# posgraph/coupe.optical_flow_based_deep_video_stabilization

Measured on AMD Instinct MI355X. Metric: stabilised frame-pairs/sec @512x512, higher is better.
Workload: dtype f32; 1 GPU; batch=8 512x512x27 frame stacks per GPU: FlowNetS-pyramid forward (5 flows) + flow resize/scale + tf_warp at 512x512; batch_per_gpu=8, height=512, width=512, cin=27, all_gather=False, vgg16_trunk=False, st_warp=none, plan_flags=0, plan_batch=0, full=False

## Files before the change

coupe/optical_flow_based_deep_video_stabilization_amd/_lib.py:

```python
from __future__ import annotations

import ctypes as C
import os

from . import build as _build

c_float_p = C.POINTER(C.c_float)
c_int32_p = C.POINTER(C.c_int32)


class VstabTensor(C.Structure):
    _fields_ = [("name", C.c_char_p), ("data", c_float_p), ("ndim", C.c_int32), ("shape", C.c_int32 * 4)]


class VstabWsEntry(C.Structure):
    _fields_ = [("name", C.c_char * 24), ("offset_bytes", C.c_int64), ("n", C.c_int32), ("h", C.c_int32),
                ("w", C.c_int32), ("c", C.c_int32), ("c_stride", C.c_int32)]


EXPORTS = {
    "vstab_create": (C.c_int, [C.POINTER(C.c_void_p), C.c_int]),
    "vstab_destroy": (None, [C.c_void_p]),
    "vstab_last_error": (C.c_char_p, [C.c_void_p]),
    "vstab_version": (C.c_char_p, []),
# ... 105 lines not shown
    "vstab_homography_fit": (C.c_int, [C.c_void_p] + [C.c_int] * 4 + [C.c_uint, C.c_double, C.c_int, C.c_int, C.c_void_p, C.c_void_p,
                                       C.c_void_p, C.c_size_t, C.c_void_p]),
    "vstab_warp_perspective_u8": (C.c_int, [C.c_void_p] + [C.c_int] * 3 + [C.c_void_p, C.c_void_p, C.c_int, C.c_int, C.c_void_p]),
    "vstab_host_xcd_remap": (C.c_int, [C.c_int] * 4 + [C.POINTER(C.c_int32)]),
    "vstab_level_sizes": (C.c_int, [C.c_int, C.c_int, c_int32_p]),
    "vstab_profile_enable": (C.c_int, [C.c_void_p, C.c_int]),
    "vstab_profile_reset": (C.c_int, [C.c_void_p]),
    "vstab_profile_read": (C.c_int, [C.c_void_p, C.POINTER(C.c_double), C.POINTER(C.c_double), C.POINTER(C.c_int)]),
    "vstab_profile_read_direct": (C.c_int, [C.c_void_p, C.POINTER(C.c_double)]),
    "vstab_profile_kernel_name": (C.c_int, [C.c_void_p, C.c_int, C.c_char_p, C.c_int]),
    "vstab_host_layer_plan": (C.c_int, [C.c_int] * 5 + [c_int32_p, C.c_int]),
    "vstab_host_layer_plan_pinned": (C.c_int, [C.c_int, C.c_uint] + [C.c_int] * 5 + [c_int32_p, C.c_int]),
    "vstab_host_pack_layer": (C.c_longlong, [C.c_int, C.c_int, c_float_p, C.POINTER(C.c_double), c_float_p,
                                             C.c_longlong]),
    "vstab_host_wdec_plan": (C.c_int, [C.c_int] * 5 + [c_int32_p, C.c_int]),
    "vstab_host_pack_wdec": (C.c_longlong, [C.c_int, c_float_p, C.POINTER(C.c_double), c_float_p, C.c_longlong]),
}

class LossLevelDesc(C.Structure):
    _fields_ = [("pf", C.c_void_p), ("grad", C.c_void_p), ("h", C.c_int), ("w", C.c_int), ("cs_pf", C.c_int), ("cs_grad", C.c_int),
                ("tv_weight", C.c_float)]


_lib = None


def lib():
    global _lib
    if _lib is None:
        path = _build.LIB
# ... 30 lines not shown
```

coupe/optical_flow_based_deep_video_stabilization_amd/build.py:

```python
from __future__ import annotations

import os
import shutil
import subprocess

HERE = os.path.dirname(os.path.abspath(__file__))
CSRC = os.path.join(HERE, "csrc")
LIB = os.path.join(HERE, "libvstab_hip.so")
SOURCES = ("conv_mfma.hip", "conv_rowwin.hip", "conv_skinny.hip", "tap_panel.hip", "wino_gemm_stream.hip", "flow_ops.hip", "sampler_ops.hip", "sampler3d_ops.hip", "nldf_ops.hip", "clip_ops.hip", "train_ops.hip", "wgrad_mfma.hip", "winograd_ops.hip", "homography_ops.hip", "pack.cpp", "conv_desc.cpp", "api.cpp", "flownet_plan.cpp", "flownet_forward.cpp", "vgg_api.cpp", "nldf_api.cpp", "train_api.cpp")
HEADERS = ("vstab_internal.h", "api_internal.h", "conv_desc.h", "flownet_plan.h", "hbm_profile.h", "tile3.h", "st_axis.h", "conv_kloop_gfx950.inc", os.path.join("..", "..", "..", "include", "vstab.h"))
FLAGS = ["--offload-arch=gfx950", "-O3", "-std=c++17", "-ffp-contract=off", "-fPIC", "-fvisibility=hidden",
         "-Wall", "-Wno-unused-result"]


def hipcc() -> str:
    for c in (os.environ.get("HIPCC"), shutil.which("hipcc"), "/opt/rocm/bin/hipcc"):
        if c and os.path.exists(c):
            return c
    raise RuntimeError("hipcc not found (set HIPCC)")


STAMP = os.path.join(HERE, "libvstab_hip.so.srchash")


def source_hash() -> str:
# ... 99 lines not shown
```

coupe/optical_flow_based_deep_video_stabilization_amd/csrc/conv_mfma.hip:

```cpp
#include <algorithm>
#include <cstdlib>

#include <hip/hip_ext.h>

#include "vstab_internal.h"

namespace vstab {

typedef float f32x4 __attribute__((ext_vector_type(4)));
typedef float f32x16 __attribute__((ext_vector_type(16)));
typedef int i32x4 __attribute__((ext_vector_type(4)));
#define VSTAB_COMMA ,
#include "conv_kloop_gfx950.inc"

#ifndef VSTAB_ABL
#define VSTAB_ABL 0
#endif

#if defined(VSTAB_HARNESS) && defined(VSTAB_STAMP)
__device__ unsigned long long g_conv_stamps[32][8 * 8192];
#define STAMP(i) do { if (threadIdx.x == 0 && sid < 8192) { g_conv_stamps[p.stamp_slot & 31][sid * 8 + (i)] = __builtin_amdgcn_s_memtime(); \
                                                          if ((i) == 0 || (i) == 3) g_conv_stamps[p.stamp_slot & 31][sid * 8 + 4 + (i) / 3] = __builtin_amdgcn_s_memrealtime(); \
                                                          if ((i) == 0) { g_conv_stamps[p.stamp_slot & 31][sid * 8 + 6] = __builtin_amdgcn_s_getreg(63492);       \
                                                                          g_conv_stamps[p.stamp_slot & 31][sid * 8 + 7] = __builtin_amdgcn_s_getreg(63508); } } } while (0)
// ... 389 lines not shown
                __builtin_amdgcn_sched_group_barrier(0x100, NRD, 1);
                __builtin_amdgcn_sched_group_barrier(0x008, G, 1);
            }
            buf ^= 1;
        }
        rd(buf, 1, fa1, fb1);
        mm(fa0, fb0);
        rd(buf, 2, fa0, fb0);
        mm(fa1, fb1);
        rd(buf, 3, fa1, fb1);
        mm(fa0, fb0);
        mm(fa1, fb1);
    }

    const bool to_slab = p.ksplit > 1;
    if (to_slab || p.out_vec4) {
        static_assert(BM * BN <= 2 * (BM + BN) * 32, "the output tile fits the operand buffers");
        __syncthreads();
        float *sC = sA;
#pragma unroll
        for (int nb = 0; nb < NB; ++nb) {
            const int cl = (wn * NB + nb) * 32 + li;
            const float bv = (!to_slab && n0 + cl < p.N) ? p.bias[n0 + cl] : 0.f;
#pragma unroll
            for (int mb = 0; mb < MB; ++mb) {
#pragma unroll
                for (int r = 0; r < 16; ++r) {
                    const int row = (wm * MB + mb) * 32 + (r & 3) + 8 * (r >> 2) + 4 * lh;
                    sC[row * BN + cl] = to_slab ? acc[mb][nb][r] : acc[mb][nb][r] + bv;
                }
            }
// ... 160 lines not shown
#else
    p.no_remap = 0;
#endif
#if defined(VSTAB_HARNESS) && defined(VSTAB_STAMP)
    p.stamp_slot = g_stamp_next++;
#endif
    p.out_vec4 = (((uintptr_t)p.out & 15) == 0 && (p.Cs_out & 3) == 0 && (p.c_off & 3) == 0) ? 1 : 0;
#ifdef VSTAB_HARNESS
    if (getenv("VSTAB_NO_VEC_EPILOGUE")) p.out_vec4 = 0;
#endif
    const int BM = (tile == TILE_64x128 || tile == TILE_64x64) ? 64 : (tile == TILE_256x32 ? 256 : 128);
    const int BN = (tile == TILE_128x128 || tile == TILE_64x128) ? 128 : ((tile == TILE_128x64 || tile == TILE_64x64) ? 64 : 32);
    if (p.in_bytes >= 0x80000000u || p.w_bytes >= 0x80000000u) return hipErrorInvalidValue;
    if (p.Npad % BN != 0 || p.SEGP % 32 != 0 || p.SEGP < p.SEG || p.NSEG < 1 || p.ksplit < 1 || p.nphase < 1 || p.nphase > 16)
        return hipErrorInvalidValue;
    if (vec4 && ((p.Cs_in & 3) || (p.SEG & 3) || (p.SEG_STRIDE & 3))) return hipErrorInvalidValue;
    if (p.ksplit > 1 && ((p.N & 3) || (p.Cs_out & 3) || (p.c_off & 3) || p.partial == nullptr || ((uintptr_t)p.partial & 15)))
        return hipErrorInvalidValue;
    dim3 grid((p.Mmax + BM - 1) / BM, p.Npad / BN, p.nphase * p.ksplit), block(256);
    const bool timed = ev_start != nullptr && ev_stop != nullptr;
#define VSTAB_LAUNCH(KERNEL, LDS)                                                                        \
    do {                                                                                                  \
        if (timed) hipExtLaunchKernelGGL(KERNEL, grid, block, LDS, stream, ev_start, ev_stop, 0, p);      \
        else KERNEL<<<grid, block, LDS, stream>>>(p);                                                     \
    } while (0)
    const bool use_dma = lds_dma_enabled();
    if (tile == TILE_128x128 && vec4 && use_dma)
        VSTAB_LAUNCH((conv_mfma_kernel<128, 128, 2, 2, true, true>), (conv_lds_bytes<128, 128>()));
    else if (tile == TILE_128x64 && vec4 && use_dma) {
        size_t lds = conv_lds_bytes<128, 64>();
// ... 37 lines not shown
    return e;
}

hipError_t launch_conv_dual(const ConvParams &pa_in, ConvTile tile_a, const ConvParams &pb_in, ConvTile tile_b, hipStream_t stream,
                            hipEvent_t ev_start, hipEvent_t ev_stop)
{
    if (!lds_dma_enabled() || tile_b != TILE_128x32 || (tile_a != TILE_128x128 && tile_a != TILE_128x64 && tile_a != TILE_64x128))
        return hipErrorNotSupported;
    ConvParams pa = pa_in, pb = pb_in;
    for (ConvParams *q : {&pa, &pb}) {
        q->no_remap = 0;
        q->out_vec4 = (((uintptr_t)q->out & 15) == 0 && (q->Cs_out & 3) == 0 && (q->c_off & 3) == 0) ? 1 : 0;
        if (q->in_bytes >= 0x80000000u || q->w_bytes >= 0x80000000u) return hipErrorInvalidValue;
        if (q->SEGP % 32 != 0 || q->SEGP < q->SEG || q->NSEG < 1 || q->ksplit < 1 || q->nphase < 1 || q->nphase > 16) return hipErrorInvalidValue;
        if ((q->Cs_in & 3) || (q->SEG & 3) || (q->SEG_STRIDE & 3)) return hipErrorInvalidValue;
        if (q->ksplit > 1 && ((q->N & 3) || (q->Cs_out & 3) || (q->c_off & 3) || q->partial == nullptr || ((uintptr_t)q->partial & 15)))
            return hipErrorInvalidValue;
    }
    const int BMa = tile_a == TILE_64x128 ? 64 : 128, BNa = tile_a == TILE_128x64 ? 64 : 128;
    if (pa.Npad % BNa != 0 || pb.Npad % 32 != 0) return hipErrorInvalidValue;
    const uint3 gA = make_uint3((unsigned)((pa.Mmax + BMa - 1) / BMa), (unsigned)(pa.Npad / BNa), (unsigned)(pa.nphase * pa.ksplit));
    const uint3 gB = make_uint3((unsigned)((pb.Mmax + 127) / 128), (unsigned)(pb.Npad / 32), (unsigned)(pb.nphase * pb.ksplit));
    const unsigned long long nA = (unsigned long long)gA.x * gA.y * gA.z, nB = (unsigned long long)gB.x * gB.y * gB.z;
    const int b_first = nA + nB > 2ull * CONV_CUS ? 1 : 0;
    const dim3 grid((unsigned)(nA + (b_first ? ((nB + 7ull) & ~7ull) : nB))), block(256);
    const bool timed = ev_start != nullptr && ev_stop != nullptr;
#define VSTAB_LAUNCH2(BM, BN, WM, WN)                                                                                                   \
    do {                                                                                                                                \
        size_t lds = std::max(conv_lds_bytes<BM, BN>(), conv_lds_bytes<128, 32>());                                                     \
        if (BN == 64 && nA > 2 * CONV_CUS && nA <= 4 * CONV_CUS && nA % (2 * CONV_CUS) == 0) lds = CONV_LDS_TWO_PER_CU;   \
// ... 13 lines not shown
```

coupe/optical_flow_based_deep_video_stabilization_amd/csrc/flownet_forward.cpp:

```cpp
#include <cmath>
#include <cstdlib>

#include "flownet_plan.h"

using namespace vstab;

static const char *UP_NAME[4] = {"upsample6_5", "upsample5_4", "upsample4_3", "upsample3_2"};

extern "C" int vstab_load_weights(vstab_ctx *ctx, const vstab_tensor *t, int count)
{
    if (!ctx) return fail(nullptr, VSTAB_E_STATE, "vstab_load_weights: ctx is NULL");
    if (!t || count <= 0) return fail(ctx, VSTAB_E_WEIGHTS, "vstab_load_weights: no tensors");
    const vstab_tensor *w1 = find(t, count, "1/W_conv2d");
    if (!w1 || w1->ndim != 4) return fail(ctx, VSTAB_E_WEIGHTS, "missing variable 1/W_conv2d");
    const int cin = w1->shape[2];
    if (cin < 1 || cin > 4096) return fail(ctx, VSTAB_E_WEIGHTS, "1/W_conv2d: bad Cin %d", cin);

    std::vector<float> host;
    auto reserve = [&](size_t n) { size_t o = (host.size() + 63) / 64 * 64; host.resize(o + n, 0.f); return o; };
    std::vector<double> scale;
    auto need = [&](const std::string &name, std::initializer_list<int> s) -> const vstab_tensor * {
        const vstab_tensor *x = find(t, count, name);
        return shape_is(x, s) ? x : nullptr;
    };
// ... 227 lines not shown
                    r.ntile_x = 0;
                }
                HIP_TRY(ctx, launch_conv_rowwin(r, stream, EV_A(0), EV_B(0)));
                PROF_NAME(0, r.MB == 2 ? "conv_rowwin_kernel<7, 2>" : "conv_rowwin_kernel<4, 1>");
                continue;
            }
        }
        if (!tickets_cleared) { HIP_TRY(ctx, hipMemsetAsync(tickets, 0, pl.bytes[B_TICKETS], stream)); tickets_cleared = true; }
        if (pl.wino[i]) {
            ConvParams q = pl.wcp[i];
            const int cin_i = e.cin;
            HIP_TRY(ctx, launch_wino_input(buf(e.in), B, pl.eh[i], pl.ew[i], in_buf(e).cs, 0, cin_i, buf(B_WINO_V), stream));
            q.in = buf(B_WINO_V); q.out = buf(B_WINO_M);
            q.wpk = dw + ctx->wino_w[i]; q.bias = dw + ctx->zero_b; q.partial = buf(B_PARTIAL);
            const int T_i = ((pl.eh[i] + 1) / 2) * ((pl.ew[i] + 1) / 2);
            const int P_i = wino_gemm_stream_positions(B, T_i, cin_i, e.cout);
            if (P_i > 0) {
                HIP_TRY(ctx, launch_wino_gemm_stream(q.in, q.wpk, q.out, B, T_i, cin_i, e.cout, P_i, stream, EV_A(i), EV_B(i)));
                PROF_NAME(i, "wino_gemm_stream_kernel");
            } else {
                HIP_TRY(ctx, launch_conv(q, pl.wtile[i], true, stream, EV_A(i), EV_B(i)));
                PROF_NAME(i, conv_kernel_name(pl.wtile[i], true));
            }
            HIP_TRY(ctx, launch_wino_output(buf(B_WINO_M), B, pl.eh[i], pl.ew[i], e.cout, dw + ctx->enc_b[i], 1, buf(e.out),
                                            out_buf(e).cs, 0, stream));
            continue;
        }
        p.in = e.in < 0 ? feats : buf(e.in);
        p.out = buf(e.out);
        p.wpk = dw + ctx->enc_w[i];
        p.bias = dw + ctx->enc_b[i];
        p.partial = buf(B_PARTIAL);
        if (pl.skinny[i]) {
            HIP_TRY(ctx, launch_conv_skinny(p, tickets, stream, EV_A(i), EV_B(i)));
            PROF_NAME(i, "conv_skinny_kernel<1, 4>");
            continue;
        }
        HIP_TRY(ctx, launch_conv(p, pl.tile[i], pl.vec4[i], stream, EV_A(i), EV_B(i)));
        PROF_NAME(i, conv_kernel_name(pl.tile[i], pl.vec4[i]));
    }
// ... 217 lines not shown
```

coupe/optical_flow_based_deep_video_stabilization_amd/csrc/flownet_plan.cpp:

```cpp
#include <cmath>
#include <cstdlib>
#include <memory>
#include <new>

#include "flownet_plan.h"

using namespace vstab;

bool level_sizes(int H, int W, int *eh, int *ew)
{
    int h = H, w = W;
    for (int i = 0; i < 10; ++i) {
        h = (h + 2 * NET[i].p - NET[i].k) / NET[i].s + 1;
        w = (w + 2 * NET[i].p - NET[i].k) / NET[i].s + 1;
        if (h < 1 || w < 1) return false;
        eh[i] = h; ew[i] = w;
    }
    for (int l = 0; l < 4; ++l)
        if ((eh[LVL_ENC[l + 1]] + 1) / 2 != eh[LVL_ENC[l]] || (ew[LVL_ENC[l + 1]] + 1) / 2 != ew[LVL_ENC[l]]) return false;
    return H >= 3 && W >= 3;
}

static double split_cost_us(long long tiles, int KT, int ks, double slab_bytes, int BN, int BM, int *ks_eff_out)
{
// ... 165 lines not shown
        }
        if (p.ksplit > 1) partial_floats = std::max(partial_floats, (size_t)p.ksplit * p.Mmax * p.Npad);
    }
    size_t wino_v = 0, wino_m = 0;
    for (int i = 0; i < 10; ++i) {
        pl.wino[i] = false;
        const Layer &e = NET[i];
        if (e.k != 3 || e.s != 1 || e.p != 1 || pl.skinny[i]) continue;
        if (ref ? !ref->wino[i] : (in_buf(e).cs != e.cin || !wino_applies(B, pl.eh[i], pl.ew[i], e.cin, e.cout))) continue;
        const int TH = (pl.eh[i] + 1) / 2, TW = (pl.ew[i] + 1) / 2;
        pl.wcp[i] = conv_desc_wino_gemm(B, pl.eh[i], pl.ew[i], e.cin, e.cout);
        {
            const long long t128 = 16LL * ((pl.wcp[i].Mmax + 127) / 128) * (e.cout / 128);
            pl.wtile[i] = t128 >= 1024 ? TILE_128x128 : TILE_128x64;
        }
        wino_v = std::max(wino_v, (size_t)B * 16 * TH * TW * e.cin);
        wino_m = std::max(wino_m, (size_t)B * 16 * TH * TW * e.cout);
        pl.wino[i] = true;
    }
    for (int l = 0; l < 4; ++l) {
        const Layer &d = dec_layer(l);
        ConvParams &p = pl.cp[10 + l];
        const int off[2] = {-1, 0};
        p = conv_desc_parity4(B, pl.buf_h(d.in), pl.buf_w(d.in), in_buf(d).cs, in_buf(d).cs, 2, off, pl.buf_h(d.out), pl.buf_w(d.out), d.cout,
                              padded_cols(d.cout), out_buf(d).cs, d.c_off, 1);
        pl.tile[10 + l] = default_tile(d.cout);
        pl.vec4[10 + l] = true;
        if (ref) { pl.tile[10 + l] = ref->tile[10 + l]; pl.skinny[10 + l] = ref->skinny[10 + l]; p.ksplit = ref->cp[10 + l].ksplit; }
        else {
            pl.tile[10 + l] = choose_tile_split(p, pl.tile[10 + l], true);
            pl.skinny[10 + l] = (flags & VSTAB_PLAN_NO_DUAL) ? choose_skinny(p, true, flags) : false;
            if (pl.skinny[10 + l]) pl.tile[10 + l] = TILE_SKINNY;
// ... 73 lines not shown
    if (chunk < 1 || !make_plan(chunk, H, W, Cin, pl)) { fail(nullptr, VSTAB_E_SHAPE, "unsupported problem %dx%dx%dx%d", B, H, W, Cin); return 0; }
    return pl.total;
}

extern "C" int vstab_set_plan_batch(vstab_ctx *ctx, int batch)
{
    if (!ctx) return fail(nullptr, VSTAB_E_STATE, "set_plan_batch: ctx is NULL");
    if (batch < 0) return fail(ctx, VSTAB_E_SHAPE, "set_plan_batch: batch must be >= 0 (0 = plan for the batch of each call)");
    ctx->plan_batch = batch;
    return VSTAB_OK;
}

extern "C" int vstab_set_plan_flags(vstab_ctx *ctx, unsigned flags)
{
    if (!ctx) return fail(nullptr, VSTAB_E_STATE, "set_plan_flags: ctx is NULL");
    if (flags & ~(unsigned)(VSTAB_PLAN_NO_SKINNY | VSTAB_PLAN_NO_DUAL | VSTAB_PLAN_NO_TAIL | VSTAB_PLAN_NO_WDEC | VSTAB_PLAN_FORCE_WDEC)) return fail(ctx, VSTAB_E_SHAPE, "set_plan_flags: unknown flag bits 0x%x", flags);
    ctx->plan_flags = flags;
    return VSTAB_OK;
}

extern "C" size_t vstab_workspace_bytes_ctx(const vstab_ctx *ctx, int B, int H, int W, int Cin)
{
    Plan pl;
    const PlanPin pin = pin_of(ctx);
    if (pin.batch > 0 && B > pin.batch) { fail(nullptr, VSTAB_E_SHAPE, "batch %d exceeds the pinned plan batch %d", B, pin.batch); return 0; }
    const int chunk = B >= 1 ? chunk_size(pin, B, H, W, Cin) : 0;
    if (chunk < 1 || !make_plan(chunk, H, W, Cin, pl, &pin)) { fail(nullptr, VSTAB_E_SHAPE, "unsupported problem %dx%dx%dx%d", B, H, W, Cin); return 0; }
    return pl.total;
}

static int workspace_layout_of(const PlanPin *pin, int chunk, int H, int W, int Cin, vstab_ws_entry *entries, int max_entries)
// ... 42 lines not shown
{
    return vstab_host_layer_plan_pinned(0, 0u, B, H, W, Cin, layer, out, cap);
}

extern "C" int vstab_host_layer_plan_pinned(int plan_batch, unsigned flags, int B, int H, int W, int Cin, int layer, int32_t *out, int cap)
{
    Plan pl;
    PlanPin pin; pin.batch = plan_batch; pin.flags = flags;
    if (!out || layer < 0 || layer > 18 || plan_batch < 0 || !make_plan(B, H, W, Cin, pl, &pin))
        return fail(nullptr, VSTAB_E_SHAPE, "layer_plan: bad arguments");
    const ConvParams &p = pl.cp[layer];
    const int need = 26 + 7 * p.nphase;
    if (cap < need) return fail(nullptr, VSTAB_E_NOMEM, "layer_plan: need %d ints", need);
    return put_desc(p, (int)pl.tile[layer], (int)pl.vec4[layer], NET[layer],
                    (layer < 10 && pl.wino[layer]) || (layer >= 10 && layer < 14 && pl.wdec[layer - 10]), out);
}

extern "C" int vstab_host_wdec_plan(int B, int H, int W, int Cin, int l, int32_t *out, int cap)
{
    Plan pl;
    if (!out || l < 0 || l > 3 || !make_plan(B, H, W, Cin, pl)) return fail(nullptr, VSTAB_E_SHAPE, "wdec_plan: bad arguments");
    const ConvParams &d = pl.cp[10 + l];
    const WdecGeom g = wdec_geom(d.Hi, d.Wi, d.Ho, d.Wo);
    const ConvParams p = conv_desc_wdec_gemm(B, g, d.Cs_in, d.N);
    const int need = 26 + 7 * 9 + 8;
    if (cap < need) return fail(nullptr, VSTAB_E_NOMEM, "wdec_plan: need %d ints", need);
    put_desc(p, (int)TILE_128x128, 1, dec_layer(l), pl.wdec[l], out);
    const int gg[8] = {g.NTy, g.NTx, g.nty[0], g.nty[1], g.nty[2], g.ntx[0], g.ntx[1], g.ntx[2]};
    for (int i = 0; i < 8; ++i) out[26 + 63 + i] = gg[i];
    return need;
// ... 44 lines not shown
```

coupe/optical_flow_based_deep_video_stabilization_amd/csrc/flownet_plan.h:

```cpp
#pragma once
#include "api_internal.h"
#include "conv_desc.h"

enum Buf { B_CONV1, B_CONCAT2, B_CONV3, B_CONCAT3, B_CONV4, B_CONCAT4, B_CONV5, B_CONCAT5, B_CONV6, B_CONV6_1, B_T,
           B_T6, B_T5, B_T4, B_T3, B_TICKETS, B_PARTIAL, B_WINO_V, B_WINO_M, N_BUF };
static_assert(B_PARTIAL == N_BUF - 3 && B_WINO_V == N_BUF - 2 && B_WINO_M == N_BUF - 1, "plan-dependent buffers must come last");

struct BufSpec { const char *name; int level, c, cs; };
constexpr BufSpec BUFS[N_BUF] = {
    {"conv1", 0, 64, 64},         {"concat2", 1, 194, 196},   {"conv3", 2, 256, 256},     {"concat3", 3, 386, 388},
    {"conv4", 4, 512, 512},       {"concat4", 5, 770, 772},   {"conv5", 6, 512, 512},     {"concat5", 7, 1026, 1028},
    {"conv6", 8, 1024, 1024},     {"conv6_1", 9, 1024, 1024}, {"pf2_taps", 1, 32, 32},    {"pf6_taps", 9, 32, 32},
    {"pf5_taps", 7, 32, 32},      {"pf4_taps", 5, 32, 32},    {"pf3_taps", 3, 32, 32},    {"tickets", -1, 0, 0},
    {"splitk", -1, 0, 0},         {"winograd_in", -1, 0, 0},  {"winograd_out", -1, 0, 0}};

enum LayerKind { L_CONV, L_DECONV, L_TAPS };
struct Layer { const char *name; LayerKind kind; int k, s, p, cin, cout, in, out, c_off; };
constexpr int N_LAYER = 19;
constexpr Layer NET[N_LAYER] = {
    {"conv1", L_CONV, 7, 2, 3, 0, 64, -1, B_CONV1, 0},              {"conv2", L_CONV, 5, 2, 2, 64, 128, B_CONV1, B_CONCAT2, 0},
    {"conv3", L_CONV, 5, 2, 2, 128, 256, B_CONCAT2, B_CONV3, 0},    {"conv3_1", L_CONV, 3, 1, 1, 256, 256, B_CONV3, B_CONCAT3, 0},
    {"conv4", L_CONV, 3, 2, 1, 256, 512, B_CONCAT3, B_CONV4, 0},    {"conv4_1", L_CONV, 3, 1, 1, 512, 512, B_CONV4, B_CONCAT4, 0},
    {"conv5", L_CONV, 3, 2, 1, 512, 512, B_CONCAT4, B_CONV5, 0},    {"conv5_1", L_CONV, 3, 1, 1, 512, 512, B_CONV5, B_CONCAT5, 0},
    {"conv6", L_CONV, 3, 2, 1, 512, 1024, B_CONCAT5, B_CONV6, 0},   {"conv6_1", L_CONV, 3, 1, 1, 1024, 1024, B_CONV6, B_CONV6_1, 0},
// ... 26 lines not shown
static_assert(net_is_consistent(), "NET and BUFS disagree");

struct Plan {
    int B, H, W, Cin;
    int eh[10], ew[10];
    size_t off[N_BUF];
    size_t bytes[N_BUF];
    size_t total;
    vstab::ConvParams cp[N_LAYER];
    vstab::ConvTile tile[N_LAYER];
    bool vec4[N_LAYER];
    bool skinny[N_LAYER];
    bool wino[10];
    vstab::ConvParams wcp[10];
    vstab::ConvTile wtile[10];
    bool wdec[4];
    vstab::ConvParams wdcp[4];
    vstab::ConvTile wdtile[4];
    vstab::WdecGeom wdg[4];
    int buf_h(int b) const { return BUFS[b].level < 0 ? 0 : eh[BUFS[b].level]; }
    int buf_w(int b) const { return BUFS[b].level < 0 ? 0 : ew[BUFS[b].level]; }
};

struct PlanPin { int batch = 0; unsigned flags = 0; };
inline PlanPin pin_of(const vstab_ctx *ctx)
{
    PlanPin pin;
    if (ctx) { pin.batch = ctx->plan_batch; pin.flags = ctx->plan_flags; }
    return pin;
}
// ... 5 lines not shown
```

coupe/optical_flow_based_deep_video_stabilization_amd/csrc/vstab_internal.h:

```cpp
#pragma once
#include <hip/hip_runtime.h>
#include <stddef.h>
#include <stdint.h>

namespace vstab {

inline int round_up_c(int a, int b) { return (a + b - 1) / b * b; }

#ifdef __HIPCC__
#define VSTAB_HD __host__ __device__
#else
#define VSTAB_HD
#endif
VSTAB_HD inline void xcd_remap_calc(unsigned Nx, unsigned Ny, unsigned Nz, unsigned lin, unsigned &bx, unsigned &by, unsigned &bz)
{
    const unsigned T = Nx * Ny * Nz;
    const unsigned q = T >> 3, r = T & 7u, c = lin & 7u, idx = lin >> 3;
    const unsigned nl = (c < r ? c * (q + 1) : r * (q + 1) + (c - r) * q) + idx;
    unsigned t2;
    if ((Ny & (Ny - 1)) == 0) { const unsigned s = 31u - (unsigned)__builtin_clz(Ny); by = nl & (Ny - 1); t2 = nl >> s; }
    else { by = nl % Ny; t2 = nl / Ny; }
    if ((Nz & (Nz - 1)) == 0) { const unsigned s = 31u - (unsigned)__builtin_clz(Nz); bz = t2 & (Nz - 1); bx = t2 >> s; }
    else { bz = t2 % Nz; bx = t2 / Nz; }
}
// ... 23 lines not shown
    float *partial;
    unsigned in_bytes;
    unsigned w_bytes;
    int B, Hi, Wi, Cs_in;
    int KH;
    int NSEG, SEG, SEGP;
    int SEG_STRIDE;
    int s_in, s_out;
    int Ho, Wo, Cs_out, c_off;
    int N, Npad;
    int act;
    int nphase, ksplit, Mmax;
    int no_remap;
    int stamp_slot;
    int out_vec4;
    ConvPhase ph[16];
};

#ifdef __HIPCC__
__device__ __forceinline__ void splitk_combine_item(const ConvParams &p, const long long idx)
{
    typedef float f32x4 __attribute__((ext_vector_type(4)));

    const int n4 = p.N >> 2;
    const long long per_phase = (long long)p.Mmax * n4;
    if (idx >= per_phase * p.nphase) return;
    const int phase = (int)(idx / per_phase);
    const long long rem = idx - phase * per_phase;
    const int m = (int)(rem / n4), c4 = (int)(rem - (long long)m * n4);
    const ConvPhase ph = p.ph[phase];
// ... 88 lines not shown
                              hipEvent_t ev_stop = nullptr);
inline int rowwin_lead(int off_x, int cs) { return ((off_x * cs) % 2 != 0) ? 1 : 0; }
inline int rowwin_segp(int off_x, int kw, int cs) { return round_up_c(rowwin_lead(off_x, cs) + kw * cs, 32); }
void pack_conv_rowwin(const float *W, const double *scale, int kh, int kw, int cin, int cout, int npad,
                      int lead, int segp, float *wpk);

hipError_t launch_wino_outgrad(const float *dy, int B, int H, int W, int Cs, int c_off, int C, float *dM, hipStream_t stream);
hipError_t launch_wino_filter_grad(const float *dU, int cin, int cout, float *dW, hipStream_t stream);
int wino_gemm_stream_positions(int B, int T, int cin, int cout);
hipError_t launch_wino_gemm_stream(const float *V, const float *wpk, float *M, int B, int T, int cin, int cout, int P, hipStream_t stream,
                                   hipEvent_t ev_start = nullptr, hipEvent_t ev_stop = nullptr);
hipError_t wino_gemm_stream_set_attributes();
hipError_t launch_wino_input(const float *x, int B, int H, int W, int Cs, int c_off, int C, float *V, hipStream_t stream,
                             bool pos_major = false);
hipError_t launch_wino_weights(const float *W, int cin, int cout, int transpose, float *Wt, hipStream_t stream);
hipError_t launch_wino_output(const float *M, int B, int Ho, int Wo, int C, const float *bias, int act, float *out, int Cs_out, int c_off,
                              hipStream_t stream);

struct WdecGeom {
    int NTy, NTx;
    int nty[3], ntx[3];
};
inline WdecGeom wdec_geom(int Hi, int Wi, int Ho, int Wo)
{
    WdecGeom g;
    g.NTy = Ho / 4 + 1; g.NTx = Wo / 4 + 1;
    g.nty[0] = g.NTy < Hi / 2 + 1 ? g.NTy : Hi / 2 + 1; g.nty[1] = g.nty[2] = g.NTy < (Hi + 1) / 2 ? g.NTy : (Hi + 1) / 2;
    g.ntx[0] = g.NTx < Wi / 2 + 1 ? g.NTx : Wi / 2 + 1; g.ntx[1] = g.ntx[2] = g.NTx < (Wi + 1) / 2 ? g.NTx : (Wi + 1) / 2;
    return g;
}
struct WdecOutArgs { const float *M; int C4; const float *bias; int act; float *out; int Ho, Wo, Cs_out, c_off; WdecGeom g; };
#ifdef __HIPCC__
// ... 248 lines not shown
```

coupe/optical_flow_based_deep_video_stabilization_amd/csrc/winograd_ops.hip:

```cpp
#include <hip/hip_runtime.h>

#include "vstab_internal.h"

namespace vstab {

typedef float f32x4 __attribute__((ext_vector_type(4)));

#ifndef VSTAB_NT_MIN_BYTES
#define VSTAB_NT_MIN_BYTES (100ll << 20)
#endif
template <bool NT>
__device__ __forceinline__ void vstore(float *p, const f32x4 v)
{
    if constexpr (NT) __builtin_nontemporal_store(v, reinterpret_cast<f32x4 *>(p));
    else *reinterpret_cast<f32x4 *>(p) = v;
}

template <bool NT>
__global__ __launch_bounds__(256) void wino_input_kernel(const float *__restrict__ x, int H, int W, int Cs, int c_off, int C4,
                                                         float *__restrict__ V, int TH, int TW, long long sample_stride, long long pos_stride)
{
    const long long idx = (long long)blockIdx.x * 256 + threadIdx.x;
    if (idx >= (long long)TH * TW * C4) return;
    const int n = blockIdx.y;
// ... 63 lines not shown
        f32x4 y0 = ((s[a][0] + s[a][1]) + s[a][2]) + bv;
        f32x4 y1 = ((s[a][1] - s[a][2]) - s[a][3]) + bv;
        float *ob = out + (((long long)n * Ho + oy) * Wo + 2 * tx) * Cs_out + c_off + c * 4;
        if (act == 3) {
            y0 += *reinterpret_cast<const f32x4 *>(ob);
            if (2 * tx + 1 < Wo) y1 += *reinterpret_cast<const f32x4 *>(ob + Cs_out);
        } else if (act) {
#pragma unroll
            for (int e = 0; e < 4; ++e) { y0[e] = fmaxf(y0[e], slope * y0[e]); y1[e] = fmaxf(y1[e], slope * y1[e]); }
        }
        *reinterpret_cast<f32x4 *>(ob) = y0;
        if (2 * tx + 1 < Wo) *reinterpret_cast<f32x4 *>(ob + Cs_out) = y1;
    }
}

__global__ __launch_bounds__(256) void wino_weight_kernel(const float *__restrict__ W, int cin, int cout, int transpose, float *__restrict__ Wt)
{
    const int K = transpose ? cout : cin, N = transpose ? cin : cout;
    const long long idx = (long long)blockIdx.x * 256 + threadIdx.x;
    if (idx >= (long long)K * N) return;
    const int k = (int)(idx / N), n = (int)(idx - (long long)k * N);
    float g[3][3];
#pragma unroll
    for (int a = 0; a < 3; ++a)
#pragma unroll
        for (int b = 0; b < 3; ++b)
            g[a][b] = transpose ? W[(((long long)(2 - a) * 3 + (2 - b)) * cin + n) * cout + k] : W[(((long long)a * 3 + b) * cin + k) * cout + n];
    float t[4][3];
#pragma unroll
    for (int b = 0; b < 3; ++b) {
// ... 167 lines not shown

hipError_t launch_wino_input(const float *x, int B, int H, int W, int Cs, int c_off, int C, float *V, hipStream_t stream, bool pos_major)
{
    if ((C & 3) || (Cs & 3) || (c_off & 3)) return hipErrorInvalidValue;
    const int TH = (H + 1) / 2, TW = (W + 1) / 2;
    const long long per = (long long)TH * TW * (C / 4), tc = (long long)TH * TW * C;
    const dim3 grid((unsigned)((per + 255) / 256), (unsigned)B);
    if ((long long)B * 16 * tc * 4 >= VSTAB_NT_MIN_BYTES)
        wino_input_kernel<true><<<grid, dim3(256), 0, stream>>>(x, H, W, Cs, c_off, C / 4, V, TH, TW, pos_major ? tc : 16 * tc, pos_major ? B * tc : tc);
    else
        wino_input_kernel<false><<<grid, dim3(256), 0, stream>>>(x, H, W, Cs, c_off, C / 4, V, TH, TW, pos_major ? tc : 16 * tc, pos_major ? B * tc : tc);
    return hipGetLastError();
}

hipError_t launch_wino_output(const float *M, int B, int Ho, int Wo, int C, const float *bias, int act, float *out, int Cs_out, int c_off,
                              hipStream_t stream)
{
    if ((C & 3) || (Cs_out & 3) || (c_off & 3)) return hipErrorInvalidValue;
    const int TH = (Ho + 1) / 2, TW = (Wo + 1) / 2;
    const long long per = (long long)TH * TW * (C / 4);
    wino_output_kernel<<<dim3((unsigned)((per + 255) / 256), (unsigned)B), dim3(256), 0, stream>>>(M, TH, TW, C / 4, bias, act, out, Ho, Wo,
                                                                                              Cs_out, c_off);
    return hipGetLastError();
}

}
```

include/vstab.h:

```cpp
#ifndef VSTAB_H
#define VSTAB_H

#include <stddef.h>
#include <stdint.h>

#ifdef __cplusplus
extern "C" {
#endif

#define VSTAB_OK          0
#define VSTAB_E_SHAPE    -1
#define VSTAB_E_ALIGN    -2
#define VSTAB_E_HIP      -3
#define VSTAB_E_NOMEM    -4
#define VSTAB_E_WEIGHTS  -5
#define VSTAB_E_STATE    -6

#if defined(__GNUC__)
#define VSTAB_API __attribute__((visibility("default")))
#else
#define VSTAB_API
#endif

typedef struct vstab_ctx vstab_ctx;
// ... 202 lines not shown
VSTAB_API int vstab_flow_mean_fill(const float *flow, int B, int h, int w, float *out, void *stream);

VSTAB_API size_t vstab_homography_workspace_bytes(int B, int H, int W, int K);
VSTAB_API int vstab_homography_fit(const float *flow, int B, int H, int W, int K, unsigned seed, double thresh, int refine,
                                   int stride, double *Hout, int32_t *inliers, void *workspace, size_t workspace_bytes,
                                   void *stream);
VSTAB_API int vstab_warp_perspective_u8(const uint8_t *src, int B, int sh, int sw, const double *Hm, uint8_t *dst, int oh, int ow,
                                        void *stream);


#define VSTAB_PLAN_NO_SKINNY 1u
#define VSTAB_PLAN_NO_DUAL 2u
#define VSTAB_PLAN_NO_TAIL 4u
#define VSTAB_PLAN_NO_WDEC 8u
#define VSTAB_PLAN_FORCE_WDEC 16u
VSTAB_API int vstab_set_plan_flags(vstab_ctx *ctx, unsigned flags);

VSTAB_API int vstab_profile_enable(vstab_ctx *ctx, int enable);
VSTAB_API int vstab_profile_reset(vstab_ctx *ctx);
VSTAB_API int vstab_profile_read(vstab_ctx *ctx, double *ms_sum15, double *flops15, int *n_forwards);
VSTAB_API int vstab_profile_read_direct(vstab_ctx *ctx, double *flops15);
VSTAB_API int vstab_profile_kernel_name(vstab_ctx *ctx, int slot, char *buf, int cap);

VSTAB_API int vstab_selftest_div_const(float d, unsigned first_bits, unsigned long long count, unsigned long long *bad_count_dev,
                                       void *stream);

VSTAB_API int vstab_trace_ranges(int on);

VSTAB_API int vstab_hbm_profile_enable(int mode);
VSTAB_API int vstab_hbm_profile_read(int slot, double *ms_sum, int *launches, double *alg_bytes_sum);

VSTAB_API int vstab_host_xcd_remap(int gx, int gy, int gz, int lin, int32_t *xyz);
VSTAB_API int vstab_level_sizes(int H, int W, int32_t *hw20);

VSTAB_API int vstab_host_layer_plan(int B, int H, int W, int Cin, int layer, int32_t *out, int cap);
VSTAB_API int vstab_host_layer_plan_pinned(int plan_batch, unsigned flags, int B, int H, int W, int Cin, int layer, int32_t *out, int cap);

VSTAB_API long long vstab_host_pack_layer(int Cin, int layer, const float *W, const double *scale,
                                          float *wpk, long long cap);

VSTAB_API int vstab_host_wdec_plan(int B, int H, int W, int Cin, int l, int32_t *out, int cap);
VSTAB_API long long vstab_host_pack_wdec(int l, const float *W, const double *scale, float *wpk, long long cap);

#ifdef __cplusplus
}
#endif
#endif
```

Baseline: 2815 frame-pairs/s.

## Store Winograd GEMM output in fragment-major layout and read it in output transform

The MFMA conv kernel now writes Winograd M tiles directly from accumulator registers in a fragment-major layout, which avoids staging the tile through shared memory. A new output-transform kernel reads 16-byte vectors in that layout. The path runs for non-streamed, non-ksplit Winograd layers, and a plan flag can restore the row-major layout. The aim is to cut LDS staging and syncs in the GEMM epilogue and to coalesce M reads, at the cost of a more complex layout and scattered output stores.

```diff
diff --git a/coupe/optical_flow_based_deep_video_stabilization_amd/_lib.py b/coupe/optical_flow_based_deep_video_stabilization_amd/_lib.py
--- a/coupe/optical_flow_based_deep_video_stabilization_amd/_lib.py
+++ b/coupe/optical_flow_based_deep_video_stabilization_amd/_lib.py
@@ -143,6 +143,9 @@
     "vstab_host_pack_layer": (C.c_longlong, [C.c_int, C.c_int, c_float_p, C.POINTER(C.c_double), c_float_p,
                                              C.c_longlong]),
     "vstab_host_wdec_plan": (C.c_int, [C.c_int] * 5 + [c_int32_p, C.c_int]),
+    "vstab_host_wino_m_plan": (C.c_int, [C.c_int, C.c_uint] + [C.c_int] * 5 + [c_int32_p]),
+    "vstab_host_wino_m_offset": (C.c_longlong, [C.c_int] * 8),
+    "vstab_host_wino_m_index": (C.c_int, [C.c_int] * 5 + [C.c_longlong, c_int32_p]),
     "vstab_host_pack_wdec": (C.c_longlong, [C.c_int, c_float_p, C.POINTER(C.c_double), c_float_p, C.c_longlong]),
 }
 
diff --git a/coupe/optical_flow_based_deep_video_stabilization_amd/build.py b/coupe/optical_flow_based_deep_video_stabilization_amd/build.py
--- a/coupe/optical_flow_based_deep_video_stabilization_amd/build.py
+++ b/coupe/optical_flow_based_deep_video_stabilization_amd/build.py
@@ -8,7 +8,7 @@
 CSRC = os.path.join(HERE, "csrc")
 LIB = os.path.join(HERE, "libvstab_hip.so")
 SOURCES = ("conv_mfma.hip", "conv_rowwin.hip", "conv_skinny.hip", "tap_panel.hip", "wino_gemm_stream.hip", "flow_ops.hip", "sampler_ops.hip", "sampler3d_ops.hip", "nldf_ops.hip", "clip_ops.hip", "train_ops.hip", "wgrad_mfma.hip", "winograd_ops.hip", "homography_ops.hip", "pack.cpp", "conv_desc.cpp", "api.cpp", "flownet_plan.cpp", "flownet_forward.cpp", "vgg_api.cpp", "nldf_api.cpp", "train_api.cpp")
-HEADERS = ("vstab_internal.h", "api_internal.h", "conv_desc.h", "flownet_plan.h", "hbm_profile.h", "tile3.h", "st_axis.h", "conv_kloop_gfx950.inc", os.path.join("..", "..", "..", "include", "vstab.h"))
+HEADERS = ("vstab_internal.h", "api_internal.h", "conv_desc.h", "flownet_plan.h", "hbm_profile.h", "tile3.h", "st_axis.h", "wino_m_layout.h", "conv_kloop_gfx950.inc", os.path.join("..", "..", "..", "include", "vstab.h"))
 FLAGS = ["--offload-arch=gfx950", "-O3", "-std=c++17", "-ffp-contract=off", "-fPIC", "-fvisibility=hidden",
          "-Wall", "-Wno-unused-result"]
 
diff --git a/coupe/optical_flow_based_deep_video_stabilization_amd/csrc/conv_mfma.hip b/coupe/optical_flow_based_deep_video_stabilization_amd/csrc/conv_mfma.hip
--- a/coupe/optical_flow_based_deep_video_stabilization_amd/csrc/conv_mfma.hip
+++ b/coupe/optical_flow_based_deep_video_stabilization_amd/csrc/conv_mfma.hip
@@ -4,6 +4,7 @@
 #include <hip/hip_ext.h>
 
 #include "vstab_internal.h"
+#include "wino_m_layout.h"
 
 namespace vstab {
 
@@ -427,7 +428,24 @@
     }
 
     const bool to_slab = p.ksplit > 1;
-    if (to_slab || p.out_vec4) {
+    if (p.m_frag && !to_slab) {
+        constexpr int LMB = MB == 2 ? 1 : 0, LNB = NB == 2 ? 1 : 0, LWN = WN == 4 ? 2 : (WN == 2 ? 1 : 0);
+        static_assert((1 << LMB) == MB && (1 << LNB) == NB && (1 << LWN) == WN, "wave tile of the fragment-major layout");
+        const int RT = (p.Mmax + BM - 1) / BM, CT = p.Npad / BN;
+        float *mt = p.out + (((long long)phase * RT + (int)bx_) * CT + (int)by_) * (BM * BN);
+#pragma unroll
+        for (int mb = 0; mb < MB; ++mb)
+#pragma unroll
+            for (int nb = 0; nb < NB; ++nb)
+#pragma unroll
+                for (int g = 0; g < 4; ++g) {
+                    const int row = (wm * MB + mb) * 32 + 8 * g + 4 * lh, col = (wn * NB + nb) * 32 + li;
+                    f32x4 v;
+#pragma unroll
+                    for (int e = 0; e < 4; ++e) v[e] = acc[mb][nb][4 * g + e] + 0.0f;
+                    *reinterpret_cast<f32x4 *>(mt + wino_m_in_tile(LMB, LNB, LWN, row, col)) = v;
+                }
+    } else if (to_slab || p.out_vec4) {
         static_assert(BM * BN <= 2 * (BM + BN) * 32, "the output tile fits the operand buffers");
         __syncthreads();
         float *sC = sA;
@@ -618,6 +636,7 @@
     if (p.in_bytes >= 0x80000000u || p.w_bytes >= 0x80000000u) return hipErrorInvalidValue;
     if (p.Npad % BN != 0 || p.SEGP % 32 != 0 || p.SEGP < p.SEG || p.NSEG < 1 || p.ksplit < 1 || p.nphase < 1 || p.nphase > 16)
         return hipErrorInvalidValue;
+    if (p.m_frag && (p.ksplit != 1 || !wino_m_layout(tile, p.Mmax, p.Npad).frag || ((uintptr_t)p.out & 15))) return hipErrorInvalidValue;
     if (vec4 && ((p.Cs_in & 3) || (p.SEG & 3) || (p.SEG_STRIDE & 3))) return hipErrorInvalidValue;
     if (p.ksplit > 1 && ((p.N & 3) || (p.Cs_out & 3) || (p.c_off & 3) || p.partial == nullptr || ((uintptr_t)p.partial & 15)))
         return hipErrorInvalidValue;
@@ -685,6 +704,7 @@
         if (q->in_bytes >= 0x80000000u || q->w_bytes >= 0x80000000u) return hipErrorInvalidValue;
         if (q->SEGP % 32 != 0 || q->SEGP < q->SEG || q->NSEG < 1 || q->ksplit < 1 || q->nphase < 1 || q->nphase > 16) return hipErrorInvalidValue;
         if ((q->Cs_in & 3) || (q->SEG & 3) || (q->SEG_STRIDE & 3)) return hipErrorInvalidValue;
+        if (q->m_frag) return hipErrorInvalidValue;
         if (q->ksplit > 1 && ((q->N & 3) || (q->Cs_out & 3) || (q->c_off & 3) || q->partial == nullptr || ((uintptr_t)q->partial & 15)))
             return hipErrorInvalidValue;
     }
diff --git a/coupe/optical_flow_based_deep_video_stabilization_amd/csrc/flownet_forward.cpp b/coupe/optical_flow_based_deep_video_stabilization_amd/csrc/flownet_forward.cpp
--- a/coupe/optical_flow_based_deep_video_stabilization_amd/csrc/flownet_forward.cpp
+++ b/coupe/optical_flow_based_deep_video_stabilization_amd/csrc/flownet_forward.cpp
@@ -265,7 +265,7 @@
             q.in = buf(B_WINO_V); q.out = buf(B_WINO_M);
             q.wpk = dw + ctx->wino_w[i]; q.bias = dw + ctx->zero_b; q.partial = buf(B_PARTIAL);
             const int T_i = ((pl.eh[i] + 1) / 2) * ((pl.ew[i] + 1) / 2);
-            const int P_i = wino_gemm_stream_positions(B, T_i, cin_i, e.cout);
+            const int P_i = pl.wstream[i];
             if (P_i > 0) {
                 HIP_TRY(ctx, launch_wino_gemm_stream(q.in, q.wpk, q.out, B, T_i, cin_i, e.cout, P_i, stream, EV_A(i), EV_B(i)));
                 PROF_NAME(i, "wino_gemm_stream_kernel");
@@ -274,7 +274,7 @@
                 PROF_NAME(i, conv_kernel_name(pl.wtile[i], true));
             }
             HIP_TRY(ctx, launch_wino_output(buf(B_WINO_M), B, pl.eh[i], pl.ew[i], e.cout, dw + ctx->enc_b[i], 1, buf(e.out),
-                                            out_buf(e).cs, 0, stream));
+                                            out_buf(e).cs, 0, stream, &pl.wml[i]));
             continue;
         }
         p.in = e.in < 0 ? feats : buf(e.in);
diff --git a/coupe/optical_flow_based_deep_video_stabilization_amd/csrc/flownet_plan.cpp b/coupe/optical_flow_based_deep_video_stabilization_amd/csrc/flownet_plan.cpp
--- a/coupe/optical_flow_based_deep_video_stabilization_amd/csrc/flownet_plan.cpp
+++ b/coupe/optical_flow_based_deep_video_stabilization_amd/csrc/flownet_plan.cpp
@@ -203,8 +203,12 @@
             const long long t128 = 16LL * ((pl.wcp[i].Mmax + 127) / 128) * (e.cout / 128);
             pl.wtile[i] = t128 >= 1024 ? TILE_128x128 : TILE_128x64;
         }
+        pl.wstream[i] = wino_gemm_stream_positions(B, TH * TW, e.cin, e.cout);
+        pl.wml[i] = WinoMLayout{0, 0, 0, 0, 0, 0};
+        if (!(flags & VSTAB_PLAN_ROWMAJOR_M) && pl.wstream[i] == 0) pl.wml[i] = wino_m_layout(pl.wtile[i], pl.wcp[i].Mmax, pl.wcp[i].Npad);
+        pl.wcp[i].m_frag = pl.wml[i].frag;
         wino_v = std::max(wino_v, (size_t)B * 16 * TH * TW * e.cin);
-        wino_m = std::max(wino_m, (size_t)B * 16 * TH * TW * e.cout);
+        wino_m = std::max(wino_m, pl.wml[i].frag ? (size_t)wino_m_floats(pl.wml[i], 16) : (size_t)B * 16 * TH * TW * e.cout);
         pl.wino[i] = true;
     }
     for (int l = 0; l < 4; ++l) {
@@ -308,7 +312,7 @@
 extern "C" int vstab_set_plan_flags(vstab_ctx *ctx, unsigned flags)
 {
     if (!ctx) return fail(nullptr, VSTAB_E_STATE, "set_plan_flags: ctx is NULL");
-    if (flags & ~(unsigned)(VSTAB_PLAN_NO_SKINNY | VSTAB_PLAN_NO_DUAL | VSTAB_PLAN_NO_TAIL | VSTAB_PLAN_NO_WDEC | VSTAB_PLAN_FORCE_WDEC)) return fail(ctx, VSTAB_E_SHAPE, "set_plan_flags: unknown flag bits 0x%x", flags);
+    if (flags & ~(unsigned)(VSTAB_PLAN_NO_SKINNY | VSTAB_PLAN_NO_DUAL | VSTAB_PLAN_NO_TAIL | VSTAB_PLAN_NO_WDEC | VSTAB_PLAN_FORCE_WDEC | VSTAB_PLAN_ROWMAJOR_M)) return fail(ctx, VSTAB_E_SHAPE, "set_plan_flags: unknown flag bits 0x%x", flags);
     ctx->plan_flags = flags;
     return VSTAB_OK;
 }
@@ -381,6 +385,42 @@
     if (cap < need) return fail(nullptr, VSTAB_E_NOMEM, "layer_plan: need %d ints", need);
     return put_desc(p, (int)pl.tile[layer], (int)pl.vec4[layer], NET[layer],
                     (layer < 10 && pl.wino[layer]) || (layer >= 10 && layer < 14 && pl.wdec[layer - 10]), out);
+}
+
+extern "C" int vstab_host_wino_m_plan(int plan_batch, unsigned flags, int B, int H, int W, int Cin, int layer, int32_t *out10)
+{
+    std::unique_ptr<Plan> pl(new (std::nothrow) Plan);
+    PlanPin pin; pin.batch = plan_batch; pin.flags = flags;
+    if (!pl || !out10 || layer < 0 || layer > 9 || plan_batch < 0 || !make_plan(B, H, W, Cin, *pl, &pin))
+        return fail(nullptr, VSTAB_E_SHAPE, "wino_m_plan: bad arguments");
+    for (int i = 0; i < 10; ++i) out10[i] = 0;
+    if (!pl->wino[layer]) return VSTAB_OK;
+    const WinoMLayout &L = pl->wml[layer];
+    const int v[10] = {1, pl->wstream[layer], L.frag, L.lmb, L.lnb, L.lwn, L.RT, L.CT, pl->wcp[layer].Mmax, pl->wcp[layer].Npad};
+    for (int i = 0; i < 10; ++i) out10[i] = v[i];
+    return VSTAB_OK;
+}
+
+static bool wino_m_args(int lmb, int lnb, int lwn, int RT, int CT, WinoMLayout &L)
+{
+    L = WinoMLayout{1, lmb, lnb, lwn, RT, CT};
+    return lmb >= 0 && lmb <= 1 && lnb >= 0 && lnb <= 1 && lwn >= 0 && lwn <= 2 && RT >= 1 && CT >= 1;
+}
+extern "C" long long vstab_host_wino_m_offset(int lmb, int lnb, int lwn, int RT, int CT, int q, int m, int c)
+{
+    WinoMLayout L;
+    if (!wino_m_args(lmb, lnb, lwn, RT, CT, L) || q < 0 || m < 0 || c < 0 || (m >> wino_m_lbm(L)) >= RT || (c >> wino_m_lbn(L)) >= CT)
+        return fail(nullptr, VSTAB_E_SHAPE, "wino_m_offset: bad arguments");
+    return wino_m_offset(L, q, m, c);
+}
+extern "C" int vstab_host_wino_m_index(int lmb, int lnb, int lwn, int RT, int CT, long long off, int32_t *qmc)
+{
+    WinoMLayout L;
+    if (!qmc || !wino_m_args(lmb, lnb, lwn, RT, CT, L) || off < 0) return fail(nullptr, VSTAB_E_SHAPE, "wino_m_index: bad arguments");
+    int q, m, c;
+    wino_m_index(L, off, q, m, c);
+    qmc[0] = q; qmc[1] = m; qmc[2] = c;
+    return VSTAB_OK;
 }
 
 extern "C" int vstab_host_wdec_plan(int B, int H, int W, int Cin, int l, int32_t *out, int cap)
diff --git a/coupe/optical_flow_based_deep_video_stabilization_amd/csrc/flownet_plan.h b/coupe/optical_flow_based_deep_video_stabilization_amd/csrc/flownet_plan.h
--- a/coupe/optical_flow_based_deep_video_stabilization_amd/csrc/flownet_plan.h
+++ b/coupe/optical_flow_based_deep_video_stabilization_amd/csrc/flownet_plan.h
@@ -1,6 +1,7 @@
 #pragma once
 #include "api_internal.h"
 #include "conv_desc.h"
+#include "wino_m_layout.h"
 
 enum Buf { B_CONV1, B_CONCAT2, B_CONV3, B_CONCAT3, B_CONV4, B_CONCAT4, B_CONV5, B_CONCAT5, B_CONV6, B_CONV6_1, B_T,
            B_T6, B_T5, B_T4, B_T3, B_TICKETS, B_PARTIAL, B_WINO_V, B_WINO_M, N_BUF };
@@ -64,6 +65,8 @@
     bool wino[10];
     vstab::ConvParams wcp[10];
     vstab::ConvTile wtile[10];
+    int wstream[10];
+    vstab::WinoMLayout wml[10];
     bool wdec[4];
     vstab::ConvParams wdcp[4];
     vstab::ConvTile wdtile[4];
diff --git a/coupe/optical_flow_based_deep_video_stabilization_amd/csrc/vstab_internal.h b/coupe/optical_flow_based_deep_video_stabilization_amd/csrc/vstab_internal.h
--- a/coupe/optical_flow_based_deep_video_stabilization_amd/csrc/vstab_internal.h
+++ b/coupe/optical_flow_based_deep_video_stabilization_amd/csrc/vstab_internal.h
@@ -61,6 +61,7 @@
     int no_remap;
     int stamp_slot;
     int out_vec4;
+    int m_frag;
     ConvPhase ph[16];
 };
 
@@ -179,8 +180,9 @@
 hipError_t launch_wino_input(const float *x, int B, int H, int W, int Cs, int c_off, int C, float *V, hipStream_t stream,
                              bool pos_major = false);
 hipError_t launch_wino_weights(const float *W, int cin, int cout, int transpose, float *Wt, hipStream_t stream);
+struct WinoMLayout;
 hipError_t launch_wino_output(const float *M, int B, int Ho, int Wo, int C, const float *bias, int act, float *out, int Cs_out, int c_off,
-                              hipStream_t stream);
+                              hipStream_t stream, const WinoMLayout *frag = nullptr);
 
 struct WdecGeom {
     int NTy, NTx;
diff --git a/coupe/optical_flow_based_deep_video_stabilization_amd/csrc/wino_m_layout.h b/coupe/optical_flow_based_deep_video_stabilization_amd/csrc/wino_m_layout.h
--- /dev/null
+++ b/coupe/optical_flow_based_deep_video_stabilization_amd/csrc/wino_m_layout.h
@@ -0,0 +1,67 @@
+#pragma once
+#include "vstab_internal.h"
+
+namespace vstab {
+
+struct WinoMLayout {
+    int frag;
+    int lmb, lnb, lwn;
+    int RT, CT;
+};
+VSTAB_HD inline int wino_m_lbm(const WinoMLayout &L) { return 5 + L.lmb + (2 - L.lwn); }
+VSTAB_HD inline int wino_m_lbn(const WinoMLayout &L) { return 5 + L.lnb + L.lwn; }
+
+VSTAB_HD inline int wino_m_in_tile(int lmb, int lnb, int lwn, int r, int c)
+{
+    const int wm = r >> (5 + lmb), mb = (r >> 5) & ((1 << lmb) - 1);
+    const int wn = c >> (5 + lnb), nb = (c >> 5) & ((1 << lnb) - 1);
+    const int wave = (wm << lwn) | wn;
+    const int piece = (((((wave << lmb) | mb) << lnb) | nb) << 2) | ((r >> 3) & 3);
+    const int lane = (((r >> 2) & 1) << 5) | (c & 31);
+    return (piece << 8) | (lane << 2) | (r & 3);
+}
+VSTAB_HD inline long long wino_m_tile_base(const WinoMLayout &L, int q, int rt, int ct)
+{
+    return (((long long)q * L.RT + rt) * L.CT + ct) << (wino_m_lbm(L) + wino_m_lbn(L));
+}
+VSTAB_HD inline long long wino_m_offset(const WinoMLayout &L, int q, int m, int c)
+{
+    const int lbm = wino_m_lbm(L), lbn = wino_m_lbn(L);
+    return wino_m_tile_base(L, q, m >> lbm, c >> lbn) + wino_m_in_tile(L.lmb, L.lnb, L.lwn, m & ((1 << lbm) - 1), c & ((1 << lbn) - 1));
+}
+VSTAB_HD inline void wino_m_index(const WinoMLayout &L, long long off, int &q, int &m, int &c)
+{
+    const int lbm = wino_m_lbm(L), lbn = wino_m_lbn(L);
+    long long t = off >> (lbm + lbn);
+    const int in = (int)(off & ((1ll << (lbm + lbn)) - 1));
+    const int ct = (int)(t % L.CT); t /= L.CT;
+    const int rt = (int)(t % L.RT); q = (int)(t / L.RT);
+    const int e = in & 3, lane = (in >> 2) & 63;
+    int piece = in >> 8;
+    const int g = piece & 3; piece >>= 2;
+    const int nb = piece & ((1 << L.lnb) - 1); piece >>= L.lnb;
+    const int mb = piece & ((1 << L.lmb) - 1); piece >>= L.lmb;
+    const int wn = piece & ((1 << L.lwn) - 1), wm = piece >> L.lwn;
+    m = (rt << lbm) + (((wm << L.lmb) | mb) << 5) + 8 * g + 4 * (lane >> 5) + e;
+    c = (ct << lbn) + (((wn << L.lnb) | nb) << 5) + (lane & 31);
+}
+inline long long wino_m_floats(const WinoMLayout &L, int P) { return wino_m_tile_base(L, P, 0, 0); }
+
+inline WinoMLayout wino_m_layout(ConvTile tile, int Mmax, int Npad)
+{
+    WinoMLayout L{0, 0, 0, 0, 0, 0};
+    switch (tile) {
+    case TILE_128x128: L.lmb = 1; L.lnb = 1; L.lwn = 1; break;
+    case TILE_128x64: L.lmb = 1; L.lnb = 0; L.lwn = 1; break;
+    case TILE_64x128: L.lmb = 1; L.lnb = 0; L.lwn = 2; break;
+    default: return L;
+    }
+    const int BM = 1 << wino_m_lbm(L), BN = 1 << wino_m_lbn(L);
+    if (Mmax < 1 || Npad < BN || Npad % BN) return L;
+    L.frag = 1;
+    L.RT = (Mmax + BM - 1) / BM;
+    L.CT = Npad / BN;
+    return L;
+}
+
+}
diff --git a/coupe/optical_flow_based_deep_video_stabilization_amd/csrc/winograd_ops.hip b/coupe/optical_flow_based_deep_video_stabilization_amd/csrc/winograd_ops.hip
--- a/coupe/optical_flow_based_deep_video_stabilization_amd/csrc/winograd_ops.hip
+++ b/coupe/optical_flow_based_deep_video_stabilization_amd/csrc/winograd_ops.hip
@@ -1,6 +1,7 @@
 #include <hip/hip_runtime.h>
 
 #include "vstab_internal.h"
+#include "wino_m_layout.h"
 
 namespace vstab {
 
@@ -101,6 +102,57 @@
     }
 }
 
+__global__ __launch_bounds__(256) void wino_output_frag_kernel(const float *__restrict__ M, const WinoMLayout L, int rows, int T, int TW, int C,
+                                                               const float *__restrict__ bias, int act, float *__restrict__ out, int Ho, int Wo,
+                                                               int Cs_out, int c_off)
+{
+    const int lane = threadIdx.x & 63, g = threadIdx.x >> 6;
+    const int cblocks = C >> 5;
+    const int rb = (int)(blockIdx.x / (unsigned)cblocks), cb = (int)(blockIdx.x - (unsigned)rb * (unsigned)cblocks);
+    const int r0 = rb * 32 + 8 * g + 4 * (lane >> 5), c = cb * 32 + (lane & 31);
+    if (r0 >= rows) return;
+    const float *mb = M + wino_m_offset(L, 0, r0, c);
+    const long long xs = wino_m_tile_base(L, 1, 0, 0);
+    f32x4 m[4][4];
+#pragma unroll
+    for (int i = 0; i < 4; ++i)
+#pragma unroll
+        for (int j = 0; j < 4; ++j) m[i][j] = *reinterpret_cast<const f32x4 *>(mb + (i * 4 + j) * xs);
+    f32x4 s[2][4];
+#pragma unroll
+    for (int j = 0; j < 4; ++j) {
+        s[0][j] = (m[0][j] + m[1][j]) + m[2][j];
+        s[1][j] = (m[1][j] - m[2][j]) - m[3][j];
+    }
+    const float bv = bias[c];
+    const float slope = act == 1 ? 0.1f : 0.0f;
+    f32x4 y[2][2];
+#pragma unroll
+    for (int a = 0; a < 2; ++a) {
+        y[a][0] = ((s[a][0] + s[a][1]) + s[a][2]) + bv;
+        y[a][1] = ((s[a][1] - s[a][2]) - s[a][3]) + bv;
+        if (act) {
+#pragma unroll
+            for (int e = 0; e < 4; ++e) { y[a][0][e] = fmaxf(y[a][0][e], slope * y[a][0][e]); y[a][1][e] = fmaxf(y[a][1][e], slope * y[a][1][e]); }
+        }
+    }
+#pragma unroll
+    for (int e = 0; e < 4; ++e) {
+        const int row = r0 + e;
+        if (row >= rows) break;
+        const int n = row / T, tile = row - n * T;
+        const int ty = tile / TW, tx = tile - ty * TW;
+#pragma unroll
+        for (int a = 0; a < 2; ++a) {
+            const int oy = 2 * ty + a;
+            if (oy >= Ho) continue;
+            float *ob = out + (((long long)n * Ho + oy) * Wo + 2 * tx) * Cs_out + c_off + c;
+            ob[0] = y[a][0][e];
+            if (2 * tx + 1 < Wo) ob[Cs_out] = y[a][1][e];
+        }
+    }
+}
+
 __global__ __launch_bounds__(256) void wino_weight_kernel(const float *__restrict__ W, int cin, int cout, int transpose, float *__restrict__ Wt)
 {
     const int K = transpose ? cout : cin, N = transpose ? cin : cout;
@@ -298,10 +350,21 @@
 }
 
 hipError_t launch_wino_output(const float *M, int B, int Ho, int Wo, int C, const float *bias, int act, float *out, int Cs_out, int c_off,
-                              hipStream_t stream)
+                              hipStream_t stream, const WinoMLayout *frag)
 {
     if ((C & 3) || (Cs_out & 3) || (c_off & 3)) return hipErrorInvalidValue;
     const int TH = (Ho + 1) / 2, TW = (Wo + 1) / 2;
+    if (frag && frag->frag) {
+        const long long rows = (long long)B * TH * TW;
+        if ((C & 31) || B < 1 || act == 3 || rows > ((long long)frag->RT << wino_m_lbm(*frag)) || C != (frag->CT << wino_m_lbn(*frag)) ||
+            rows >= 0x7fffffffLL || ((uintptr_t)M & 15))
+            return hipErrorInvalidValue;
+        const long long blocks = ((rows + 31) / 32) * (C / 32);
+        if (blocks >= 0x7fffffffLL) return hipErrorInvalidValue;
+        wino_output_frag_kernel<<<dim3((unsigned)blocks), dim3(256), 0, stream>>>(M, *frag, (int)rows, TH * TW, TW, C, bias, act, out, Ho, Wo, Cs_out,
+                                                                                 c_off);
+        return hipGetLastError();
+    }
     const long long per = (long long)TH * TW * (C / 4);
     wino_output_kernel<<<dim3((unsigned)((per + 255) / 256), (unsigned)B), dim3(256), 0, stream>>>(M, TH, TW, C / 4, bias, act, out, Ho, Wo,
                                                                                               Cs_out, c_off);
diff --git a/include/vstab.h b/include/vstab.h
--- a/include/vstab.h
+++ b/include/vstab.h
@@ -240,6 +240,7 @@
 #define VSTAB_PLAN_NO_TAIL 4u
 #define VSTAB_PLAN_NO_WDEC 8u
 #define VSTAB_PLAN_FORCE_WDEC 16u
+#define VSTAB_PLAN_ROWMAJOR_M 32u
 VSTAB_API int vstab_set_plan_flags(vstab_ctx *ctx, unsigned flags);
 
 VSTAB_API int vstab_profile_enable(vstab_ctx *ctx, int enable);
@@ -261,6 +262,9 @@
 
 VSTAB_API int vstab_host_layer_plan(int B, int H, int W, int Cin, int layer, int32_t *out, int cap);
 VSTAB_API int vstab_host_layer_plan_pinned(int plan_batch, unsigned flags, int B, int H, int W, int Cin, int layer, int32_t *out, int cap);
+VSTAB_API int vstab_host_wino_m_plan(int plan_batch, unsigned flags, int B, int H, int W, int Cin, int layer, int32_t *out10);
+VSTAB_API long long vstab_host_wino_m_offset(int lmb, int lnb, int lwn, int RT, int CT, int q, int m, int c);
+VSTAB_API int vstab_host_wino_m_index(int lmb, int lnb, int lwn, int RT, int CT, long long off, int32_t *qmc);
 
 VSTAB_API long long vstab_host_pack_layer(int Cin, int layer, const float *W, const double *scale,
                                           float *wpk, long long cap);
```

New measurement: 2815 frame-pairs/s (median of 2 runs). No clear change (+0.0%).
